# kevlar-dev/kevlar

Measured on AMD Instinct MI355X. Metric: reads/sec through count+novel (3 samples, k=31), higher is better.
Workload: dtype u64 hash / u8 counters

## Files before the change

kevlar_amd/csrc/kv_skm_bucket_device.h:

```cpp
#pragma once
#include "kv_skm_emit_device.h"

#define SKM_MAX_ABL 8
struct SkmAblSet {
    int n, ctrl_max;
    const uint64_t *keys[SKM_MAX_ABL];
    const uint8_t *cnts[SKM_MAX_ABL];
    const uint32_t *bstart[SKM_MAX_ABL], *bcount[SKM_MAX_ABL];
    uint32_t maxv[SKM_MAX_ABL];
};

namespace {

#define SKM_THREADS3 512
#define SKM_BUCKETS_PER_TICKET 8u
#define SKM_MAXPROBE 48
#define SKM_LOOSE_WGS 1024

#define SKM_STEP_MASK 62u
#define SKM_PROBE_STEP(h) ((((h) >> 20) & SKM_STEP_MASK) | 1u)
template <int TS>
__device__ __forceinline__ uint32_t skm_slot0(uint32_t sh) { return (TS & (TS - 1)) == 0 ? sh & (uint32_t)(TS - 1) : __umulhi(sh, (uint32_t)TS); }
template <int TS>
__device__ __forceinline__ uint32_t skm_step_of(uint32_t sh) { return (TS & (TS - 1)) == 0 ? SKM_PROBE_STEP(sh) : (((sh >> 2) & 62u) | 1u); }
template <int TS>
__device__ __forceinline__ uint32_t skm_slot_next(uint32_t slot, uint32_t step)
{
    if ((TS & (TS - 1)) == 0) return (slot + step) & (uint32_t)(TS - 1);
    slot += step;
    return slot >= (uint32_t)TS ? slot - (uint32_t)TS : slot;
}
template <int KW, int TS>
struct SkmTable {
    unsigned long long key[KW][TS];
};

template <int KW, int TS>
__device__ __forceinline__ void skm_table_clear(SkmTable<KW, TS> &tb)
{
    for (uint32_t i = threadIdx.x; i < TS; i += blockDim.x) {
        tb.key[0][i] = SKM_EMPTY;
        if (KW == 2) tb.key[KW - 1][i] = SKM_EMPTY;
    }
}

template <int KW, int TS>
__device__ __forceinline__ int skm_table_insert(SkmTable<KW, TS> &tb, const SkmKey<KW> &c)
{
    const uint32_t sh = skm_slot_hash<KW>(c);
    uint32_t slot = skm_slot0<TS>(sh);
    const uint32_t step = skm_step_of<TS>(sh);
    for (int probe = 0; probe < SKM_MAXPROBE; ++probe) {
        const unsigned long long old0 = atomicCAS(&tb.key[0][slot], SKM_EMPTY, (unsigned long long)c.w[0]);
        if (old0 == SKM_EMPTY || old0 == c.w[0]) {
            if (KW == 1) return (int)slot;
            const unsigned long long old1 = atomicCAS(&tb.key[KW - 1][slot], SKM_EMPTY, (unsigned long long)c.w[KW - 1]);
            if (old1 == SKM_EMPTY || old1 == c.w[KW - 1]) return (int)slot;
        }
        slot = skm_slot_next<TS>(slot, step);
    }
    return -1;
}

template <int KW, int TS>
__device__ __forceinline__ int skm_table_find(const SkmTable<KW, TS> &tb, const SkmKey<KW> &c)
{
    const uint32_t sh = skm_slot_hash<KW>(c);
    uint32_t slot = skm_slot0<TS>(sh);
    const uint32_t step = skm_step_of<TS>(sh);
    for (int probe = 0; probe < SKM_MAXPROBE; ++probe) {
        const unsigned long long k0 = tb.key[0][slot];
        if (k0 == SKM_EMPTY) return -1;
        if (k0 == c.w[0] && (KW == 1 || tb.key[KW - 1][slot] == c.w[KW - 1])) return (int)slot;
        slot = skm_slot_next<TS>(slot, step);
    }
    return -1;
}

template <int KW, int TS>
__device__ __forceinline__ SkmKey<KW> skm_table_key(const SkmTable<KW, TS> &tb, uint32_t slot)
{
    SkmKey<KW> c;
    c.w[0] = tb.key[0][slot];
    if (KW == 2) c.w[KW - 1] = tb.key[KW - 1][slot];
    return c;
}
template <int KW, int TS>
__device__ __forceinline__ SkmKey<KW> skm_table_take(SkmTable<KW, TS> &tb, uint32_t slot)
{
    const SkmKey<KW> c = skm_table_key(tb, slot);
    tb.key[0][slot] = SKM_EMPTY;
    if (KW == 2) tb.key[KW - 1][slot] = SKM_EMPTY;
    return c;
}

template <int KW>
__device__ __forceinline__ SkmKey<KW> skm_key_load(const uint64_t *keys, uint64_t e, bool live = true)
{
    SkmKey<KW> c;
    c.w[0] = live ? keys[e * KW] : SKM_EMPTY;
    if (KW == 2) c.w[KW - 1] = live ? keys[e * KW + (KW - 1)] : SKM_EMPTY;
    return c;
}
template <int KW>
__device__ __forceinline__ void skm_key_store(uint64_t *keys, uint64_t e, const SkmKey<KW> &c)
{
    keys[e * KW] = c.w[0];
    if (KW == 2) keys[e * KW + (KW - 1)] = c.w[KW - 1];
}
// ... 37 lines not shown
}

template <int TS, typename Body>
__device__ __forceinline__ void skm_for_occupied(const unsigned long long *key0, uint16_t *queue_all, uint32_t queue_stride, Body body, const uint32_t *skip = nullptr)
{
    const uint32_t wave = threadIdx.x >> 6, lane = threadIdx.x & 63, nwaves = blockDim.x >> 6;
    uint16_t *queue = queue_all + wave * queue_stride;
    const uint32_t per_wave = TS / nwaves;
    const uint32_t s_end = (wave + 1) * per_wave;
    uint32_t qn = 0;
    for (uint32_t s0 = wave * per_wave;; s0 += 64) {
        const bool last = s0 >= s_end;
        if (!last) {
            const uint32_t slot = s0 + lane;
            const bool occ = key0[slot] != SKM_EMPTY && !(skip && ((skip[slot >> 5] >> (slot & 31u)) & 1u));
            const unsigned long long ballot = __ballot(occ);
            if (occ) __hip_atomic_store(&queue[qn + (uint32_t)__popcll(ballot & ((1ull << lane) - 1ull))], (uint16_t)slot, __ATOMIC_RELAXED, __HIP_MEMORY_SCOPE_WAVEFRONT);
            qn += (uint32_t)__popcll(ballot);
            __builtin_amdgcn_fence(__ATOMIC_ACQ_REL, "wavefront");
            __builtin_amdgcn_wave_barrier();
        }
        if (qn >= 64 || (last && qn > 0)) {
            const uint32_t take = min(qn, 64u);
            qn -= take;
            if (lane < take) body((uint32_t)__hip_atomic_load(&queue[qn + lane], __ATOMIC_RELAXED, __HIP_MEMORY_SCOPE_WAVEFRONT));
            __builtin_amdgcn_fence(__ATOMIC_ACQ_REL, "wavefront");
            __builtin_amdgcn_wave_barrier();
        }
        if (last) break;
    }
}

#define SKM_UNIT 4

__device__ __forceinline__ uint64_t skm_shfl64(uint64_t v, uint32_t src)
{
    const uint32_t lo = (uint32_t)__shfl((int)(uint32_t)v, (int)src), hi = (uint32_t)__shfl((int)(uint32_t)(v >> 32), (int)src);
    return (uint64_t)lo | ((uint64_t)hi << 32);
}

template <int KW, bool WANT_POS>
__device__ __forceinline__ void skm_walk_loose(const SkmGeom &sg, bool alone, const SkmKey<KW> &kmer, uint64_t hdr, uint32_t owner,
                                               uint64_t pos0, uint32_t j0, uint32_t u, uint32_t lane, int recw)
{
    const unsigned long long need = __ballot(alone);
    if (!need) return;
    const uint64_t posu = WANT_POS ? pos0 : skm_hdr_pos_of(skm_shfl64(hdr, owner), j0 + u);
    unsigned long long first = 0;
    if (lane == 0) first = atomicAdd(&sg.ctr[SKM_CTR_LOOSE], (unsigned long long)__popcll(need));
    first = skm_shfl64(first, 0);
    if (alone) {
        const unsigned long long idx = first + (unsigned long long)__popcll(need & ((1ull << lane) - 1ull));
        uint64_t one[3] = {kmer.w[0], KW == 2 ? kmer.w[KW - 1] : 0ull, 0ull};
        if (idx < sg.loose_cap) skm_store_record(sg.loose + idx * (uint64_t)recw, skm_header(posu, 1u, 0u), one, sg.nbw);
        else sg.ctr[SKM_CTR_FAIL] = 1;
    }
}

template <int KW, bool WANT_POS, int FK = 0, bool COMPACT = false, typename Body>
__device__ __forceinline__ void skm_walk_bucket(const SkmGeom &sg, uint32_t b, uint32_t *sbits_all, Body body)
{
    static_assert(!COMPACT || (KW == 1 && !WANT_POS), "compact records: one-word keys, no positions");
    constexpr uint32_t G = SKM_UNIT;
    const uint32_t lane = threadIdx.x & 63, wave = threadIdx.x >> 6, nwaves = blockDim.x >> 6;
    uint32_t *sbits = sbits_all + wave * sg.sbw;
    const int k = FK ? FK : sg.k, recw = COMPACT ? 2 : (FK ? 1 + KW + 1 : sg.recw);
    auto load = [&](const uint64_t *rec, uint64_t &hdr, uint64_t &b0, uint64_t &b1, uint64_t &b2) {
        if (COMPACT) {
            typedef uint64_t u64x2a __attribute__((ext_vector_type(2), aligned(16)));
            const u64x2a both = *(const u64x2a *)rec;
            b0 = both.x; b1 = skm_c_b1(both.y); hdr = skm_header(0ull, skm_c_n(both.y), 0u, skm_c_rev(both.y));
        } else {
            hdr = rec[0]; b0 = rec[1]; b1 = rec[2];
            if (KW == 2) b2 = rec[3];
        }
    };
    const uint32_t *cnt2 = sg.cnt2 + (uint64_t)b * sg.nwg2;
    uint32_t p = wave;
    uint32_t g = p / sg.nwg2, sgm = p - g * sg.nwg2;
    uint64_t hdr = 0, b0 = 0, b1 = 0, b2 = 0;
    {
        const uint32_t at = min(g * 64u + lane, sg.cap2 - 1u);
        const uint64_t *rec = sg.seg2 + (((uint64_t)b * sg.nwg2 + sgm) * sg.cap2 + at) * (uint64_t)recw;
        load(rec, hdr, b0, b1, b2);
    }
    uint32_t maxc = 0;
    for (uint32_t s2 = 0; s2 < sg.nwg2; ++s2) maxc = max(maxc, cnt2[s2]);
    for (;;) {
        if (g * 64u >= maxc) break;
        const uint32_t NR = cnt2[sgm], i = g * 64u + lane;
        const uint32_t nk = i < NR ? skm_hdr_n(hdr) : 0u;
        const uint32_t nu = (nk + G - 1u) / G;
        uint32_t incl = nu;
#pragma unroll
        for (int d = 1; d < 64; d <<= 1) {
            const uint32_t up = __shfl_up(incl, d);
            if (lane >= d) incl += up;
        }
        const uint32_t total = __shfl(incl, 63), excl = incl - nu;
        const uint32_t exnk = excl | (nk << 16);
        const uint32_t nwords = (total >> 5) + 2u;
        for (uint32_t wd = lane; wd < nwords; wd += 64) sbits[wd] = 0;
        __builtin_amdgcn_fence(__ATOMIC_RELEASE, "wavefront");
        __builtin_amdgcn_wave_barrier();
        if (nu) atomicOr(&sbits[excl >> 5], 1u << (excl & 31));
        __builtin_amdgcn_fence(__ATOMIC_ACQ_REL, "wavefront");
        __builtin_amdgcn_wave_barrier();
        uint32_t before = 0;
        for (uint32_t t0 = 0; t0 < total; t0 += 64) {
            const uint64_t starts = (uint64_t)__hip_atomic_load(&sbits[t0 >> 5], __ATOMIC_RELAXED, __HIP_MEMORY_SCOPE_WAVEFRONT) |
                                    ((uint64_t)__hip_atomic_load(&sbits[(t0 >> 5) + 1], __ATOMIC_RELAXED, __HIP_MEMORY_SCOPE_WAVEFRONT) << 32);
            const uint32_t t = t0 + lane;
            const uint32_t owner = (before + (uint32_t)__popcll(starts & ((2ull << lane) - 1ull)) - 1u) & 63u;
            before += (uint32_t)__popcll(starts);
            const uint32_t oe = (uint32_t)__shfl((int)exnk, (int)owner);
            const uint64_t o0 = skm_shfl64(b0, owner), o1 = skm_shfl64(b1, owner);
            const uint64_t o2 = KW == 2 ? skm_shfl64(b2, owner) : 0ull;
            const uint64_t oh = WANT_POS ? skm_shfl64(hdr, owner) : 0ull;
            const uint32_t j0 = t < total ? (t - (oe & 0xffffu)) * G : 0u;
            const uint32_t cnt = t < total ? min(G, (oe >> 16) - j0) : 0u;
            SkmKey<KW> fw = skm_kmer_of<KW>(o0, o1, o2, j0, k);
            const uint32_t tail = (uint32_t)skm_window64(o0, o1, o2, j0 + (uint32_t)k);
            uint64_t pos0 = 0;
            int step = 1;
            if (WANT_POS) {
                const bool rv = skm_hdr_rev(oh) != 0u;
                pos0 = skm_hdr_pos(oh) + (rv ? skm_hdr_n(oh) - 1u - j0 : j0);
                step = rv ? -1 : 1;
            }
#pragma unroll
            for (uint32_t u = 0; u < G; ++u) {
                if (u) { SkmKey<KW> other = fw; skm_roll<KW>(fw, other, (tail >> (2u * (u - 1u))) & 3u, k); }
                const uint64_t posu = pos0 + (uint64_t)(int64_t)(step * (int)u);
                bool alone = false;
                if (u < cnt) alone = body(fw, posu);
                skm_walk_loose<KW, WANT_POS>(sg, alone, fw, hdr, owner, posu, j0, u, lane, sg.lrecw);
            }
        }
        __builtin_amdgcn_wave_barrier();
        p += nwaves;
        g = p / sg.nwg2; sgm = p - g * sg.nwg2;
        if (g * 64u >= maxc) break;
        if (g * 64u + lane < cnt2[sgm]) {
            const uint64_t *rec = sg.seg2 + (((uint64_t)b * sg.nwg2 + sgm) * sg.cap2 + g * 64u + lane) * (uint64_t)recw;
            load(rec, hdr, b0, b1, b2);
        }
    }
}

template <int CTR>
__device__ __forceinline__ uint32_t skm_first_bucket(const SkmGeom &sg) { return (uint32_t)atomicAdd(&sg.ctr[CTR], 1ull) * sg.bpt; }

template <int CTR, bool FAIL_ENDS, bool ESTIMATE>
__device__ __forceinline__ void skm_next_bucket(const SkmGeom &sg, uint32_t b, uint32_t taken, uint32_t &next)
{
    if ((b + 1u) & (sg.bpt - 1u)) next = b + 1u;
    else if (taken + 1 >= sg.quota3 || (FAIL_ENDS && __hip_atomic_load(&sg.ctr[SKM_CTR_FAIL], __ATOMIC_RELAXED, __HIP_MEMORY_SCOPE_AGENT) != 0)) next = 0xffffffffu;
    else {
        const unsigned long long ticket = atomicAdd(&sg.ctr[CTR], 1ull);
        next = (uint32_t)ticket * sg.bpt;
        if (ESTIMATE) {
            const unsigned long long done = ticket * sg.bpt;
            if (done * 50ull >= sg.n_buckets) {
                const unsigned long long now = __hip_atomic_load(&sg.ctr[SKM_CTR_LOOSE], __ATOMIC_RELAXED, __HIP_MEMORY_SCOPE_AGENT), start = sg.ctr[SKM_CTR_LOOSE_S12];
                if (now > start && (now - start) * 25ull > done * sg.bucket_kmers) sg.ctr[SKM_CTR_FAIL] = 1;
            }
        }
    }
}

__device__ __forceinline__ uint64_t skm_loose_len(const SkmGeom &sg)
{
    const unsigned long long n = sg.ctr[SKM_CTR_LOOSE];
    return n > sg.loose_cap ? sg.loose_cap : n;
}

template <int KW, typename Body>
__device__ __forceinline__ void skm_loose_walk_wave(const SkmGeom &sg, Body body)
{
    const unsigned long long n = skm_loose_len(sg);
// ... 2 lines not shown
    const uint64_t total_waves = (uint64_t)gridDim.x * (blockDim.x >> 6), wave_id = (uint64_t)blockIdx.x * (blockDim.x >> 6) + (threadIdx.x >> 6);
    const uint32_t per = (uint32_t)min((unsigned long long)64, max((unsigned long long)1, (n + total_waves - 1) / total_waves));
    for (uint64_t i0 = wave_id * per; i0 < n; i0 += total_waves * per) {
        const uint64_t i = i0 + lane;
        const bool have = lane < per && i < n;
        const uint64_t *rec = sg.loose + (have ? i : 0) * (uint64_t)sg.lrecw;
        uint64_t bw[3];
#pragma unroll
        for (int t = 0; t < 3; ++t) bw[t] = (have && t < sg.nbw) ? rec[1 + t] : 0ull;
        const uint64_t hdr = have ? rec[0] : 0ull;
        const uint32_t nk = skm_hdr_n(hdr);
        body(skm_first_kmer<KW>(bw, k), nk == 1, hdr, 0u);
        unsigned long long longer = __ballot(nk > 1);
        while (longer) {
            const uint32_t src = (uint32_t)__ffsll((long long)longer) - 1u;
            longer &= longer - 1ull;
            const uint64_t b0 = skm_shfl64(bw[0], src), b1 = skm_shfl64(bw[1], src), b2 = skm_shfl64(bw[2], src), h_src = skm_shfl64(hdr, src);
            const uint32_t nk_src = (uint32_t)__shfl((int)nk, (int)src);
            for (uint32_t j0 = 0; j0 < nk_src; j0 += 64) {
                const uint32_t j = j0 + lane;
                const bool live = j < nk_src;
                body(skm_kmer_of<KW>(b0, b1, b2, live ? j : 0u, k), live, h_src, live ? j : 0u);
            }
        }
    }
}

__host__ __device__ inline uint32_t skm_wave_scratch_words(uint32_t sbw) { return sbw > 64u ? sbw : 64u; }

#define SKM_K2_WAVES 6
#define SKM_TS51 2560
#define SKM_TS31 4096
#define SKM_LIST_MAX 4096u
template <int KW, int TS, bool FORCE_LOOSE, int FK, bool COMPACT = false>
__global__ __launch_bounds__(SKM_THREADS3, KW == 2 ? SKM_K2_WAVES : 6) void k_skm_count(SkmGeom sg, const SketchDev *__restrict__ sk,
                                                           const SketchDev *__restrict__ mask, ConsumeFilter f, BinGeom g)
{
    static_assert((uint32_t)TS <= SKM_LIST_MAX, "a bucket's distinct list (one entry per occupied slot) must fit what k_skm_novel_list takes");
    constexpr bool PL = FK != 0;
    __shared__ SkmTable<KW, TS> tb;
    __shared__ uint32_t cnt[PL ? TS / 2 : TS];
    __shared__ uint32_t next_bucket;
    __shared__ uint32_t abl_cur, abl_b0, abl_prev;
    __shared__ uint32_t dl_cur, dl_b0;
    extern __shared__ __attribute__((aligned(16))) uint32_t dyn[];
    const uint32_t ns = (uint32_t)(g.T * g.C);
    uint32_t *lut = dyn, *cur = dyn + (PL ? 1024 : 256), *scratch = cur + ((ns + 3u) & ~3u);
    uint64_t *P1 = (uint64_t *)dyn, *P2 = P1 + 256;
    for (uint32_t s = threadIdx.x; s < ns; s += SKM_THREADS3) cur[s] = 0;
    if (threadIdx.x < 256) {
        if (PL) { P1[threadIdx.x] = skm_ascii4_times(threadIdx.x, MM_C1); P2[threadIdx.x] = skm_ascii4_times(threadIdx.x, MM_C2); }
        else lut[threadIdx.x] = skm_ascii4(threadIdx.x);
    }
    const HashParams hp = FK ? make_hash_params(FK, f.hp.hashfam) : f.hp;
    uint64_t n_added = 0, n_distinct = 0;
    const uint32_t cap1 = (uint32_t)g.cap1;
    uint32_t *my_seg = g.gbuf1 + (uint64_t)blockIdx.x * g.cap1;
    const uint64_t seg_stride = (uint64_t)g.nwgA * g.cap1;
    auto emit = [&](int t, uint64_t bin, uint32_t wgt) {
        const uint32_t slice = (uint32_t)(bin >> g.sbits);
        const uint32_t c = g.F == 1 ? slice : __umulhi(slice, g.recipF);
        const uint32_t sidx = (uint32_t)t * (uint32_t)g.C + c;
        const uint32_t item = ((slice - c * (uint32_t)g.F) << g.sbits) | ((uint32_t)bin & ((1u << g.sbits) - 1u)) | ((wgt - 1u) << BIN_W_SHIFT);
        const uint32_t pos = atomicAdd(&cur[sidx], 1u);
        if (pos < cap1) my_seg[sidx * seg_stride + pos] = item;
        else spill_item(g, t, bin, wgt);
    };
    skm_table_clear(tb);
    for (uint32_t i = threadIdx.x; i < (PL ? TS / 2 : TS); i += SKM_THREADS3) cnt[i] = 0;
    if (threadIdx.x == 0) { next_bucket = skm_first_bucket<SKM_CTR_TICKET_COUNT>(sg); abl_cur = 0; abl_b0 = 0; abl_prev = 0xffffffffu; dl_cur = 0; dl_b0 = 0; }
    auto abl_close = [&]() {
        if (sg.abl_keys && abl_prev != 0xffffffffu) {
            const bool fits = abl_cur <= sg.abl_cap_wg;
            sg.abl_bstart[abl_prev] = blockIdx.x * sg.abl_cap_wg + abl_b0;
            sg.abl_bcount[abl_prev] = fits ? abl_cur - abl_b0 : 0u;
        }
        if (sg.dl_keys && abl_prev != 0xffffffffu) {
            sg.dl_bstart[abl_prev] = blockIdx.x * sg.dl_cap_wg + dl_b0;
            sg.dl_bcount[abl_prev] = dl_cur - dl_b0;
        }
    };
    for (uint32_t taken = 0; taken < sg.quota3; ++taken) {
        __syncthreads();
        const uint32_t b = next_bucket;
        if (b >= sg.n_buckets) break;
        __syncthreads();
        if (threadIdx.x == 0) {
            abl_close();
            abl_prev = b; abl_b0 = abl_cur; dl_b0 = dl_cur;
            skm_next_bucket<SKM_CTR_TICKET_COUNT, true, true>(sg, b, taken, next_bucket);
        }
        skm_walk_bucket<KW, false, FK, COMPACT>(sg, b, scratch, [&](const SkmKey<KW> &c, uint64_t) {
            const bool forced = FORCE_LOOSE && sg.force_loose && ((c.w[0] * 0x9e3779b97f4a7c15ull) >> 58) == 0;
            const int slot = skm_cacheable<KW>(c) && !forced ? skm_table_insert(tb, c) : -1;
            if (slot >= 0) {
                if (PL) atomicAdd(&cnt[(uint32_t)slot >> 1], 1u << (((uint32_t)slot & 1u) * 16u));
                else atomicAdd(&cnt[slot], 1u);
            }
            return slot < 0;
        });
        __syncthreads();
        skm_for_occupied<TS>(tb.key[0], (uint16_t *)scratch, skm_wave_scratch_words(sg.sbw) * 2u, [&](uint32_t slot) {
            const SkmKey<KW> c = skm_table_take(tb, slot);
            uint32_t seen;
            if (PL) {
                const uint32_t sh = (slot & 1u) * 16u;
                seen = (cnt[slot >> 1] >> sh) & 0xffffu;
                atomicSub(&cnt[slot >> 1], seen << sh);
            } else {
                seen = cnt[slot];
                cnt[slot] = 0;
            }
            n_distinct += 1;
            uint64_t h;
            if constexpr (PL) h = skm_key_hash_pl<KW, FK>(c, P1, P2);
            else h = skm_key_hash<KW>(c, lut, hp);
            if (sg.dl_keys) skm_dl_push<KW>(sg, &dl_cur, (uint64_t)blockIdx.x * sg.dl_cap_wg, sg.dl_cap_wg, c, h);
            uint32_t added;
            if (g.fast4 && !f.use_mask) {
                const bool pass = !f.use_band || (h >= f.band_lo && h < f.band_hi);
                added = pass ? seen : 0u;
                if (pass) {
                    const double hd = kv_fastmod_hd(h);
                    uint32_t bin[4];
#pragma unroll
                    for (int t = 0; t < 4; ++t) bin[t] = kv_fastmod32(h, hd, (uint32_t)g.tsize[t], g.tmagic[t]);
                    uint32_t left = min(seen, 255u);
                    const uint32_t omask = (1u << g.sbits) - 1u, stride32 = (uint32_t)seg_stride;
                    while (left) {
                        const uint32_t wgt = min(left, BIN_W_MAX), wbits = (wgt - 1u) << BIN_W_SHIFT;
#pragma unroll
                        for (int t = 0; t < 4; ++t) {
                            const uint32_t slice = bin[t] >> g.sbits;
                            const uint32_t c = g.F == 1 ? slice : __umulhi(slice, g.recipF);
                            const uint32_t sidx = (uint32_t)t * (uint32_t)g.C + c;
                            const uint32_t item = ((slice - c * (uint32_t)g.F) << g.sbits) | (bin[t] & omask) | wbits;
                            const uint32_t pos = atomicAdd(&cur[sidx], 1u);
                            if (pos < cap1) my_seg[sidx * stride32 + pos] = item;
                            else spill_item(g, t, (uint64_t)bin[t], wgt);
                        }
                        left -= wgt;
                    }
                }
            } else {
                added = skm_count_kmer(h, seen, sk, mask, f, g.T, emit);
            }
            n_added += added;
            if (sg.abl_keys) {
                const bool want = added >= 2u;
                const uint32_t at = skm_wave_reserve(&abl_cur, want);
                if (want && at < sg.abl_cap_wg) {
                    const uint64_t e = (uint64_t)blockIdx.x * sg.abl_cap_wg + at;
                    skm_key_store<KW>(sg.abl_keys, e, c);
                    sg.abl_cnts[e] = (uint8_t)min(added, 255u);
                }
            }
        });
    }
    __syncthreads();
    if (threadIdx.x == 0) {
        abl_close();
        if (sg.dl_keys && dl_cur > sg.dl_cap_wg) atomicAdd(&sg.ctr[SKM_CTR_DL_RAN_OUT], 1ull);
    }
    for (uint32_t s = threadIdx.x; s < ns; s += SKM_THREADS3)
        g.gcnt1[(uint64_t)s * g.nwgA + blockIdx.x] = (uint32_t)min((uint64_t)cur[s], g.cap1);
    n_added = wave_sum_u64(n_added);
    n_distinct = wave_sum_u64(n_distinct);
    if ((threadIdx.x & 63) == 0 && n_added) atomicAdd(&g.ctr[BIN_CTR_ADDED], (unsigned long long)n_added);
    if ((threadIdx.x & 63) == 0 && n_distinct) atomicAdd(&sg.ctr[SKM_CTR_DISTINCT], (unsigned long long)n_distinct);
}

template <int KW>
__global__ __launch_bounds__(256) void k_skm_loose_count(SkmGeom sg, const SketchDev *__restrict__ sk,
                                                         const SketchDev *__restrict__ mask, ConsumeFilter f, BinGeom g)
{
    __shared__ uint32_t lut[256];
    if (sg.ctr[SKM_CTR_FAIL] != 0) return;
    lut[threadIdx.x] = skm_ascii4(threadIdx.x);
    __syncthreads();
    const int k = sg.k;
    uint64_t n_added = 0;
    skm_loose_walk_wave<KW>(sg, [&](const SkmKey<KW> &fw, bool live, uint64_t, uint32_t) {
        uint64_t h = 0;
        bool pass = false;
        if (live) {
            h = skm_key_hash<KW>(skm_canonical<KW>(fw, skm_revcomp<KW>(fw, k)), lut, f.hp);
            pass = consume_filter_pass(f, mask, h);
// ... 514 lines not shown
```

kevlar_amd/csrc/kv_skm.hip:

```cpp
#include <algorithm>
#include <cmath>

#include "kv_binned.h"
#include "kv_novel_device.h"
#include "kv_skm_device.h"
#include "kv_skm_emit_device.h"
#include "kv_skm_bucket_device.h"

namespace {

template <typename F> KvInst<F> skm_inst(F *fn, const char *name) { return kv_inst(fn, name); }
#define SKM_INST(...) skm_inst(__VA_ARGS__, #__VA_ARGS__)
KvPerStream<KvLaunched> g_skm_launched;
void skm_launched_begin(hipStream_t st) { g_skm_launched.get(st).begin(); }
template <typename F> F *skm_launching(const KvInst<F> &k, hipStream_t st)
{
    g_skm_launched.get(st).note(k.name);
    return k.fn;
}

struct SkmCarve {
    unsigned char *base;
    size_t total = 0;
    explicit SkmCarve(void *arena = nullptr) : base((unsigned char *)arena) {}
// ... 441 lines not shown
                if (al.mem) (void)hipFree(al.mem);
                al.mem = nullptr; al.bytes = 0;
                if (kv_hip_malloc(&al.mem, need) == hipSuccess) al.bytes = need;
                else (void)hipGetLastError();
            }
            if (al.mem) {
                skm_list_lay(SkmCarve(al.mem), cap_wg * nwg3, sg.kw, sg.n_buckets, &al.keys, &al.cnts, &al.bstart, &al.bcount);
                KV_HIP(skm_list_zero(al.bstart, al.bcount, st));
                al.k = k; al.m = sg.m; al.kw = sg.kw; al.C1 = sg.C1; al.F2 = sg.F2; al.fbits = sg.fbits; al.n_buckets = sg.n_buckets;
                al.nwg = nwg3; al.cap_wg = cap_wg; al.cap_total = cap_wg * nwg3;
                skm_abl_attach(al, sg);
                abl_new = true;
            }
        }
    }
    bool dl_new = false;
    const char *dl_env = kv_knob("KV_SKM_DL");
    if (s->scan_hint && !(dl_env && atoi(dl_env) == 0)) {
        const double frac = std::min(1.0, std::max(0.3, s->skm_distinct * 1.15));
        const uint64_t cap_wg = std::min<uint64_t>((uint64_t)((double)n_kmers * frac * 1.6 / nwg3) + 4096, 0xfffffff0ull / nwg3);
        const bool worth = (dl_env && atoi(dl_env) == 1) || s->scan_steady || idx.builds > 1 || idx.dl.bytes >= SkmDistinctList::bytes(cap_wg * nwg3, sg.kw, sg.n_buckets);
        const int lrc = worth ? idx.list.carve(idx.dl, cap_wg * nwg3, sg.kw, sg.n_buckets, (uint32_t)cap_wg, 0, 0, st) : KV_ERR_CAPACITY;
        if (lrc != KV_OK && lrc != KV_ERR_CAPACITY) return lrc;
        if (lrc == KV_OK) { idx.list.attach(sg); dl_new = true; }
        else (void)hipGetLastError();
    }
    {
        KvProfScope prof("k_skm_count");
        const uint32_t ns = (uint32_t)(plan.g.T * plan.g.C);
        const bool fixed_k = !sg.force_loose && !kv_knob("KV_SKM_ANY_K") && (uint64_t)sg.nwg2 * sg.cap2 * (uint64_t)sg.ncap < 65536ull;
        auto kernel = sg.kw == 1 ? (sg.force_loose ? SKM_INST(k_skm_count<1, 4096, true, 0>) : SKM_INST(k_skm_count<1, 4096, false, 0>))
                                 : (sg.force_loose ? SKM_INST(k_skm_count<2, 2048, true, 0>) : SKM_INST(k_skm_count<2, 2048, false, 0>));
        bool pl = false;
        if (sg.k == 31 && sg.recw == 3 && fixed_k) { kernel = SKM_INST(k_skm_count<1, SKM_TS31, false, 31>); pl = true; }
        if (sg.compact) {
            kernel = sg.force_loose ? SKM_INST(k_skm_count<1, 4096, true, 0, true>) : SKM_INST(k_skm_count<1, 4096, false, 0, true>);
            pl = false;
            if (sg.k == 31 && fixed_k) { kernel = SKM_INST(k_skm_count<1, SKM_TS31, false, 31, true>); pl = true; }
        }
        if (sg.k == 51 && sg.recw == 4 && fixed_k) { kernel = SKM_INST(k_skm_count<2, SKM_TS51, false, 51>); pl = true; }
        const size_t lds = ((pl ? 1024 : 256) + ((ns + 3u) & ~3u) + (size_t)(SKM_THREADS3 / 64) * skm_wave_scratch_words(sg.sbw)) * 4;
        hipLaunchKernelGGL(skm_launching(kernel, st), dim3(nwg3), dim3(SKM_THREADS3), lds, st, sg, (const SketchDev *)s->d_desc, d_mask, filter, plan.g);
    }
    {
        KvProfScope prof("k_skm_loose_count");
        skm_launch_loose(SKM_INST(k_skm_loose_count<1>), SKM_INST(k_skm_loose_count<2>), st, sg, s->d_desc, d_mask, filter, plan.g);
    }
    KV_HIP(hipGetLastError());
    hipLaunchKernelGGL(k_skm_forward_flag, dim3(1), dim3(1), 0, st, sg.ctr, plan.g.ctr);
    KV_HIP(hipGetLastError());
    skm_abl_detach(sg);
    SkmDistinctList::detach(sg);
    const int rc = kv_bin_finish(s, plan, true, 0, n_added);
    if (abl_new) s->abl.valid = rc == KV_OK;
    {
        unsigned long long sc[SKM_CTR_DL_RAN_OUT + 1] = {0};
        const bool got = hipMemcpy(sc, sg.ctr, sizeof(sc), hipMemcpyDeviceToHost) == hipSuccess;
        idx.dl_valid = dl_new && got && rc == KV_OK && sc[SKM_CTR_DL_RAN_OUT] == 0;
        if (dl_new && kv_knob("KV_SKM_VERBOSE")) fprintf(stderr, "[kv_skm] distinct list: %s (%llu workgroups ran out of %u entries)\n", idx.dl_valid ? "kept" : "dropped", sc[SKM_CTR_DL_RAN_OUT], idx.list.cap_wg);
        if (got && n_kmers) {
            const double alone = skm_outside_tables(sc) / (double)n_kmers;
            const double distinct = (double)sc[SKM_CTR_DISTINCT] / (double)n_kmers + alone;
            s->skm_off = rc != KV_OK || alone > 0.03 || distinct > 0.45;
            s->skm_off_kmers = (distinct > 0.45 || rc == KV_ERR_CAPACITY) ? n_kmers : 0;
            s->skm_distinct = distinct;
            { std::lock_guard<std::mutex> glk(g_skm_mu); g_skm_last_distinct = distinct; }
            if (kv_knob("KV_SKM_VERBOSE"))
                fprintf(stderr, "[kv_skm] batch of %llu k-mers: %.1f%% distinct, %.2f%% outside the LDS tables, %llu of %llu records (%d bytes each) outside their segments%s\n",
                        (unsigned long long)n_kmers, 100 * distinct, 100 * alone, sc[SKM_CTR_LOOSE_S12], sc[SKM_CTR_RECORDS], 8 * sg.recw,
                        s->skm_off ? " -> next batches take the plain partition" : "");
        }
    }
    if (rc != KV_OK) {
        idx.drop(SkmIndex::BATCH | SkmIndex::MEX_SCAN);
// ... 480 lines not shown
```

Before: 1.060 billion.

## Re-read kernel arguments from kernarg segment to cut register pressure; unroll probes

Inside the per-bucket loops the kernel now gets a fresh pointer to its kernarg segment, hidden behind an empty asm barrier. Geometry, filter and bin fields are then reloaded as scalar loads instead of being kept live in registers across the whole kernel. The hash-table insert and find loops are rewritten with a single exit and an explicit clang unroll count. The aim is to lower SGPR/VGPR pressure and spills at the 6-waves launch bound and to let probes issue back to back. The cost is that it depends on the argument block layout matching a hand-written struct, which is checked only by a static_assert.

```diff
diff --git a/kevlar_amd/csrc/kv_skm_bucket_device.h b/kevlar_amd/csrc/kv_skm_bucket_device.h
--- a/kevlar_amd/csrc/kv_skm_bucket_device.h
+++ b/kevlar_amd/csrc/kv_skm_bucket_device.h
@@ -1,4 +1,5 @@
 #pragma once
+#include <cstddef>
 #include "kv_skm_emit_device.h"
 
 #define SKM_MAX_ABL 8
@@ -15,6 +16,7 @@
 #define SKM_THREADS3 512
 #define SKM_BUCKETS_PER_TICKET 8u
 #define SKM_MAXPROBE 48
+#define SKM_PROBE_UNROLL(KW) ((KW) == 1 ? 8 : 4)
 #define SKM_LOOSE_WGS 1024
 
 #define SKM_STEP_MASK 62u
@@ -50,16 +52,19 @@
     const uint32_t sh = skm_slot_hash<KW>(c);
     uint32_t slot = skm_slot0<TS>(sh);
     const uint32_t step = skm_step_of<TS>(sh);
+    int at = -1;
+#pragma clang loop unroll_count(SKM_PROBE_UNROLL(KW))
     for (int probe = 0; probe < SKM_MAXPROBE; ++probe) {
         const unsigned long long old0 = atomicCAS(&tb.key[0][slot], SKM_EMPTY, (unsigned long long)c.w[0]);
-        if (old0 == SKM_EMPTY || old0 == c.w[0]) {
-            if (KW == 1) return (int)slot;
+        bool mine = old0 == SKM_EMPTY || old0 == c.w[0];
+        if (KW == 2 && mine) {
             const unsigned long long old1 = atomicCAS(&tb.key[KW - 1][slot], SKM_EMPTY, (unsigned long long)c.w[KW - 1]);
-            if (old1 == SKM_EMPTY || old1 == c.w[KW - 1]) return (int)slot;
-        }
+            mine = old1 == SKM_EMPTY || old1 == c.w[KW - 1];
+        }
+        if (mine) { at = (int)slot; break; }
         slot = skm_slot_next<TS>(slot, step);
     }
-    return -1;
+    return at;
 }
 
 template <int KW, int TS>
@@ -68,13 +73,15 @@
     const uint32_t sh = skm_slot_hash<KW>(c);
     uint32_t slot = skm_slot0<TS>(sh);
     const uint32_t step = skm_step_of<TS>(sh);
+    int at = -1;
+#pragma clang loop unroll_count(SKM_PROBE_UNROLL(KW))
     for (int probe = 0; probe < SKM_MAXPROBE; ++probe) {
         const unsigned long long k0 = tb.key[0][slot];
-        if (k0 == SKM_EMPTY) return -1;
-        if (k0 == c.w[0] && (KW == 1 || tb.key[KW - 1][slot] == c.w[KW - 1])) return (int)slot;
+        if (k0 == SKM_EMPTY) break;
+        if (k0 == c.w[0] && (KW == 1 || tb.key[KW - 1][slot] == c.w[KW - 1])) { at = (int)slot; break; }
         slot = skm_slot_next<TS>(slot, step);
     }
-    return -1;
+    return at;
 }
 
 template <int KW, int TS>
@@ -360,6 +367,18 @@
 #define SKM_TS51 2560
 #define SKM_TS31 4096
 #define SKM_LIST_MAX 4096u
+struct SkmCountArgs { SkmGeom sg; const SketchDev *sk, *mask; ConsumeFilter f; BinGeom g; };
+static_assert(alignof(SkmGeom) == 8 && alignof(ConsumeFilter) == 8 && alignof(BinGeom) == 8 &&
+              offsetof(SkmCountArgs, g) == sizeof(SkmGeom) + 2 * sizeof(void *) + sizeof(ConsumeFilter),
+              "SkmCountArgs must lie as k_skm_count's argument block does");
+template <typename Args>
+__device__ __forceinline__ const Args *skm_args_again()
+{
+    typedef const __attribute__((address_space(4))) Args *ArgsPtr;
+    ArgsPtr p = (ArgsPtr)__builtin_amdgcn_kernarg_segment_ptr();
+    asm volatile("" : "+s"(p));
+    return (const Args *)p;
+}
 template <int KW, int TS, bool FORCE_LOOSE, int FK, bool COMPACT = false>
 __global__ __launch_bounds__(SKM_THREADS3, KW == 2 ? SKM_K2_WAVES : 6) void k_skm_count(SkmGeom sg, const SketchDev *__restrict__ sk,
                                                            const SketchDev *__restrict__ mask, ConsumeFilter f, BinGeom g)
@@ -418,8 +437,9 @@
             abl_prev = b; abl_b0 = abl_cur; dl_b0 = dl_cur;
             skm_next_bucket<SKM_CTR_TICKET_COUNT, true, true>(sg, b, taken, next_bucket);
         }
-        skm_walk_bucket<KW, false, FK, COMPACT>(sg, b, scratch, [&](const SkmKey<KW> &c, uint64_t) {
-            const bool forced = FORCE_LOOSE && sg.force_loose && ((c.w[0] * 0x9e3779b97f4a7c15ull) >> 58) == 0;
+        const SkmGeom &sw = skm_args_again<SkmCountArgs>()->sg;
+        skm_walk_bucket<KW, false, FK, COMPACT>(sw, b, scratch, [&](const SkmKey<KW> &c, uint64_t) {
+            const bool forced = FORCE_LOOSE && sw.force_loose && ((c.w[0] * 0x9e3779b97f4a7c15ull) >> 58) == 0;
             const int slot = skm_cacheable<KW>(c) && !forced ? skm_table_insert(tb, c) : -1;
             if (slot >= 0) {
                 if (PL) atomicAdd(&cnt[(uint32_t)slot >> 1], 1u << (((uint32_t)slot & 1u) * 16u));
@@ -428,6 +448,10 @@
             return slot < 0;
         });
         __syncthreads();
+        const SkmCountArgs &ka = *skm_args_again<SkmCountArgs>();
+        const SkmGeom &sd = ka.sg; const ConsumeFilter &fd = ka.f; const BinGeom &gd = ka.g;
+        const uint32_t cap1d = (uint32_t)gd.cap1, stride32 = (uint32_t)((uint64_t)gd.nwgA * gd.cap1);
+        uint32_t *seg_d = gd.gbuf1 + (uint64_t)blockIdx.x * gd.cap1;
         skm_for_occupied<TS>(tb.key[0], (uint16_t *)scratch, skm_wave_scratch_words(sg.sbw) * 2u, [&](uint32_t slot) {
             const SkmKey<KW> c = skm_table_take(tb, slot);
             uint32_t seen;
@@ -443,29 +467,29 @@
             uint64_t h;
             if constexpr (PL) h = skm_key_hash_pl<KW, FK>(c, P1, P2);
             else h = skm_key_hash<KW>(c, lut, hp);
-            if (sg.dl_keys) skm_dl_push<KW>(sg, &dl_cur, (uint64_t)blockIdx.x * sg.dl_cap_wg, sg.dl_cap_wg, c, h);
+            if (sd.dl_keys) skm_dl_push<KW>(sd, &dl_cur, (uint64_t)blockIdx.x * sd.dl_cap_wg, sd.dl_cap_wg, c, h);
             uint32_t added;
-            if (g.fast4 && !f.use_mask) {
-                const bool pass = !f.use_band || (h >= f.band_lo && h < f.band_hi);
+            if (gd.fast4 && !fd.use_mask) {
+                const bool pass = !fd.use_band || (h >= fd.band_lo && h < fd.band_hi);
                 added = pass ? seen : 0u;
                 if (pass) {
                     const double hd = kv_fastmod_hd(h);
                     uint32_t bin[4];
 #pragma unroll
-                    for (int t = 0; t < 4; ++t) bin[t] = kv_fastmod32(h, hd, (uint32_t)g.tsize[t], g.tmagic[t]);
+                    for (int t = 0; t < 4; ++t) bin[t] = kv_fastmod32(h, hd, (uint32_t)gd.tsize[t], gd.tmagic[t]);
                     uint32_t left = min(seen, 255u);
-                    const uint32_t omask = (1u << g.sbits) - 1u, stride32 = (uint32_t)seg_stride;
+                    const uint32_t omask = (1u << gd.sbits) - 1u;
                     while (left) {
                         const uint32_t wgt = min(left, BIN_W_MAX), wbits = (wgt - 1u) << BIN_W_SHIFT;
 #pragma unroll
                         for (int t = 0; t < 4; ++t) {
-                            const uint32_t slice = bin[t] >> g.sbits;
-                            const uint32_t c = g.F == 1 ? slice : __umulhi(slice, g.recipF);
-                            const uint32_t sidx = (uint32_t)t * (uint32_t)g.C + c;
-                            const uint32_t item = ((slice - c * (uint32_t)g.F) << g.sbits) | (bin[t] & omask) | wbits;
+                            const uint32_t slice = bin[t] >> gd.sbits;
+                            const uint32_t c = gd.F == 1 ? slice : __umulhi(slice, gd.recipF);
+                            const uint32_t sidx = (uint32_t)t * (uint32_t)gd.C + c;
+                            const uint32_t item = ((slice - c * (uint32_t)gd.F) << gd.sbits) | (bin[t] & omask) | wbits;
                             const uint32_t pos = atomicAdd(&cur[sidx], 1u);
-                            if (pos < cap1) my_seg[sidx * stride32 + pos] = item;
-                            else spill_item(g, t, (uint64_t)bin[t], wgt);
+                            if (pos < cap1d) seg_d[sidx * stride32 + pos] = item;
+                            else spill_item(gd, t, (uint64_t)bin[t], wgt);
                         }
                         left -= wgt;
                     }
@@ -474,13 +498,13 @@
                 added = skm_count_kmer(h, seen, sk, mask, f, g.T, emit);
             }
             n_added += added;
-            if (sg.abl_keys) {
+            if (sd.abl_keys) {
                 const bool want = added >= 2u;
                 const uint32_t at = skm_wave_reserve(&abl_cur, want);
-                if (want && at < sg.abl_cap_wg) {
-                    const uint64_t e = (uint64_t)blockIdx.x * sg.abl_cap_wg + at;
-                    skm_key_store<KW>(sg.abl_keys, e, c);
-                    sg.abl_cnts[e] = (uint8_t)min(added, 255u);
+                if (want && at < sd.abl_cap_wg) {
+                    const uint64_t e = (uint64_t)blockIdx.x * sd.abl_cap_wg + at;
+                    skm_key_store<KW>(sd.abl_keys, e, c);
+                    sd.abl_cnts[e] = (uint8_t)min(added, 255u);
                 }
             }
         });
```

Measured after the change: 1.068 billion, median of 4. About the same (+0.7%).

## Combine duplicate compact super-k-mer records before k-mer insertion in count kernel

Applied to the files above, without the earlier changes.

For the k=31 compact-record path, each bucket's two-word records are first deduplicated in a record hash table that overlays the k-mer table in LDS, and each copy count becomes a weight. The walk then compacts away duplicate records per wave and inserts each distinct record's k-mers once, adding the weight to the counter. This targets the repeated LDS atomic inserts caused by identical reads at high coverage. In exchange it adds a pre-pass with atomics, extra syncs and more LDS, and falls back to unweighted walking when a bucket has more than two 64-record groups per wave or the record table overflows.

```diff
diff --git a/kevlar_amd/csrc/kv_skm.hip b/kevlar_amd/csrc/kv_skm.hip
--- a/kevlar_amd/csrc/kv_skm.hip
+++ b/kevlar_amd/csrc/kv_skm.hip
@@ -497,14 +497,16 @@
         auto kernel = sg.kw == 1 ? (sg.force_loose ? SKM_INST(k_skm_count<1, 4096, true, 0>) : SKM_INST(k_skm_count<1, 4096, false, 0>))
                                  : (sg.force_loose ? SKM_INST(k_skm_count<2, 2048, true, 0>) : SKM_INST(k_skm_count<2, 2048, false, 0>));
         bool pl = false;
+        bool rc = false;
         if (sg.k == 31 && sg.recw == 3 && fixed_k) { kernel = SKM_INST(k_skm_count<1, SKM_TS31, false, 31>); pl = true; }
         if (sg.compact) {
             kernel = sg.force_loose ? SKM_INST(k_skm_count<1, 4096, true, 0, true>) : SKM_INST(k_skm_count<1, 4096, false, 0, true>);
             pl = false;
-            if (sg.k == 31 && fixed_k) { kernel = SKM_INST(k_skm_count<1, SKM_TS31, false, 31, true>); pl = true; }
+            if (sg.k == 31 && fixed_k) { kernel = SKM_INST(k_skm_count<1, SKM_TS31, false, 31, true>); pl = true; rc = true; }
         }
         if (sg.k == 51 && sg.recw == 4 && fixed_k) { kernel = SKM_INST(k_skm_count<2, SKM_TS51, false, 51>); pl = true; }
-        const size_t lds = ((pl ? 1024 : 256) + ((ns + 3u) & ~3u) + (size_t)(SKM_THREADS3 / 64) * skm_wave_scratch_words(sg.sbw)) * 4;
+        const size_t lds = ((pl ? 1024 : 256) + ((ns + 3u) & ~3u) + (size_t)(SKM_THREADS3 / 64) * skm_wave_scratch_words(sg.sbw)) * 4 +
+                           (rc ? SKM_RC_LDS_WORDS * 4 : 0);
         hipLaunchKernelGGL(skm_launching(kernel, st), dim3(nwg3), dim3(SKM_THREADS3), lds, st, sg, (const SketchDev *)s->d_desc, d_mask, filter, plan.g);
     }
     {
diff --git a/kevlar_amd/csrc/kv_skm_bucket_device.h b/kevlar_amd/csrc/kv_skm_bucket_device.h
--- a/kevlar_amd/csrc/kv_skm_bucket_device.h
+++ b/kevlar_amd/csrc/kv_skm_bucket_device.h
@@ -1,4 +1,6 @@
 #pragma once
+#include <cstddef>
+#include <type_traits>
 #include "kv_skm_emit_device.h"
 
 #define SKM_MAX_ABL 8
@@ -45,7 +47,7 @@
 }
 
 template <int KW, int TS>
-__device__ __forceinline__ int skm_table_insert(SkmTable<KW, TS> &tb, const SkmKey<KW> &c)
+__device__ __forceinline__ int skm_table_insert(SkmTable<KW, TS> &tb, const SkmKey<KW> &c, bool *claimed = nullptr)
 {
     const uint32_t sh = skm_slot_hash<KW>(c);
     uint32_t slot = skm_slot0<TS>(sh);
@@ -53,9 +55,15 @@
     for (int probe = 0; probe < SKM_MAXPROBE; ++probe) {
         const unsigned long long old0 = atomicCAS(&tb.key[0][slot], SKM_EMPTY, (unsigned long long)c.w[0]);
         if (old0 == SKM_EMPTY || old0 == c.w[0]) {
-            if (KW == 1) return (int)slot;
+            if (KW == 1) {
+                if (claimed) *claimed = old0 == SKM_EMPTY;
+                return (int)slot;
+            }
             const unsigned long long old1 = atomicCAS(&tb.key[KW - 1][slot], SKM_EMPTY, (unsigned long long)c.w[KW - 1]);
-            if (old1 == SKM_EMPTY || old1 == c.w[KW - 1]) return (int)slot;
+            if (old1 == SKM_EMPTY || old1 == c.w[KW - 1]) {
+                if (claimed) *claimed = old1 == SKM_EMPTY;
+                return (int)slot;
+            }
         }
         slot = skm_slot_next<TS>(slot, step);
     }
@@ -178,6 +186,12 @@
 }
 
 #define SKM_UNIT 4
+#define SKM_RC_GROUPS 2u
+#define SKM_RC_LDS_WORDS ((SKM_THREADS3 / 64) * SKM_RC_GROUPS * 64u / 2u + 4u)
+struct SkmRecWeights {
+    const uint16_t *all;
+    bool hold;
+};
 
 __device__ __forceinline__ uint64_t skm_shfl64(uint64_t v, uint32_t src)
 {
@@ -185,13 +199,32 @@
     return (uint64_t)lo | ((uint64_t)hi << 32);
 }
 
-template <int KW, bool WANT_POS>
+template <int KW, bool WANT_POS, bool WEIGHTED = false>
 __device__ __forceinline__ void skm_walk_loose(const SkmGeom &sg, bool alone, const SkmKey<KW> &kmer, uint64_t hdr, uint32_t owner,
-                                               uint64_t pos0, uint32_t j0, uint32_t u, uint32_t lane, int recw)
+                                               uint64_t pos0, uint32_t j0, uint32_t u, uint32_t lane, int recw, uint32_t wt = 1u)
 {
     const unsigned long long need = __ballot(alone);
     if (!need) return;
     const uint64_t posu = WANT_POS ? pos0 : skm_hdr_pos_of(skm_shfl64(hdr, owner), j0 + u);
+    if constexpr (WEIGHTED) {
+        const uint32_t mine = alone ? wt : 0u;
+        uint32_t incl = mine;
+#pragma unroll
+        for (int d = 1; d < 64; d <<= 1) {
+            const uint32_t up = __shfl_up(incl, d);
+            if (lane >= (uint32_t)d) incl += up;
+        }
+        const uint32_t total = __shfl(incl, 63);
+        unsigned long long first = 0;
+        if (lane == 0) first = atomicAdd(&sg.ctr[SKM_CTR_LOOSE], (unsigned long long)total);
+        first = skm_shfl64(first, 0) + (incl - mine);
+        uint64_t one[3] = {kmer.w[0], KW == 2 ? kmer.w[KW - 1] : 0ull, 0ull};
+        for (uint32_t c = 0; c < mine; ++c) {
+            if (first + c < sg.loose_cap) skm_store_record(sg.loose + (first + c) * (uint64_t)recw, skm_header(posu, 1u, 0u), one, sg.nbw);
+            else sg.ctr[SKM_CTR_FAIL] = 1;
+        }
+        return;
+    }
     unsigned long long first = 0;
     if (lane == 0) first = atomicAdd(&sg.ctr[SKM_CTR_LOOSE], (unsigned long long)__popcll(need));
     first = skm_shfl64(first, 0);
@@ -203,12 +236,16 @@
     }
 }
 
-template <int KW, bool WANT_POS, int FK = 0, bool COMPACT = false, typename Body>
-__device__ __forceinline__ void skm_walk_bucket(const SkmGeom &sg, uint32_t b, uint32_t *sbits_all, Body body)
+template <int KW, bool WANT_POS, int FK = 0, bool COMPACT = false, typename Body, typename Wts = std::nullptr_t>
+__device__ __forceinline__ void skm_walk_bucket(const SkmGeom &sg, uint32_t b, uint32_t *sbits_all, Body body, Wts wts = nullptr)
 {
     static_assert(!COMPACT || (KW == 1 && !WANT_POS), "compact records: one-word keys, no positions");
+    constexpr bool WEIGHTED = !std::is_same<Wts, std::nullptr_t>::value;
+    static_assert(!WEIGHTED || COMPACT, "weights: compact records (n < 64, so at most 1024 units in front of a record: exnk below)");
     constexpr uint32_t G = SKM_UNIT;
-    const uint32_t lane = threadIdx.x & 63, wave = threadIdx.x >> 6, nwaves = blockDim.x >> 6;
+    uint32_t tid = threadIdx.x;
+    if constexpr (WEIGHTED) asm volatile("" : "+v"(tid));
+    const uint32_t lane = tid & 63, wave = tid >> 6, nwaves = blockDim.x >> 6;
     uint32_t *sbits = sbits_all + wave * sg.sbw;
     const int k = FK ? FK : sg.k, recw = COMPACT ? 2 : (FK ? 1 + KW + 1 : sg.recw);
     auto load = [&](const uint64_t *rec, uint64_t &hdr, uint64_t &b0, uint64_t &b1, uint64_t &b2) {
@@ -232,10 +269,30 @@
     }
     uint32_t maxc = 0;
     for (uint32_t s2 = 0; s2 < sg.nwg2; ++s2) maxc = max(maxc, cnt2[s2]);
-    for (;;) {
+    for (uint32_t r = 0;; ++r) {
         if (g * 64u >= maxc) break;
         const uint32_t NR = cnt2[sgm], i = g * 64u + lane;
-        const uint32_t nk = i < NR ? skm_hdr_n(hdr) : 0u;
+        uint32_t wt = 1u;
+        bool live = i < NR;
+        if constexpr (WEIGHTED) {
+            if (wts.hold) {
+                wt = wts.all[(wave * SKM_RC_GROUPS + r) * 64u + lane];
+                const unsigned long long keep = __ballot(live && wt != 0u);
+                uint16_t *from = (uint16_t *)sbits;
+                if (live && wt != 0u)
+                    __hip_atomic_store(&from[__builtin_amdgcn_mbcnt_hi((uint32_t)(keep >> 32), __builtin_amdgcn_mbcnt_lo((uint32_t)keep, 0u))], (uint16_t)lane,
+                                       __ATOMIC_RELAXED, __HIP_MEMORY_SCOPE_WAVEFRONT);
+                __builtin_amdgcn_fence(__ATOMIC_ACQ_REL, "wavefront");
+                __builtin_amdgcn_wave_barrier();
+                live = lane < (uint32_t)__popcll(keep);
+                const uint32_t src = live ? (uint32_t)__hip_atomic_load(&from[lane], __ATOMIC_RELAXED, __HIP_MEMORY_SCOPE_WAVEFRONT) : lane;
+                __builtin_amdgcn_fence(__ATOMIC_ACQ_REL, "wavefront");
+                __builtin_amdgcn_wave_barrier();
+                hdr = skm_shfl64(hdr, src); b0 = skm_shfl64(b0, src); b1 = skm_shfl64(b1, src);
+                wt = (uint32_t)__shfl((int)wt, (int)src);
+            }
+        }
+        const uint32_t nk = live ? skm_hdr_n(hdr) : 0u;
         const uint32_t nu = (nk + G - 1u) / G;
         uint32_t incl = nu;
 #pragma unroll
@@ -244,7 +301,7 @@
             if (lane >= d) incl += up;
         }
         const uint32_t total = __shfl(incl, 63), excl = incl - nu;
-        const uint32_t exnk = excl | (nk << 16);
+        const uint32_t exnk = WEIGHTED ? excl | (nk << 10) | (wt << 16) : excl | (nk << 16);
         const uint32_t nwords = (total >> 5) + 2u;
         for (uint32_t wd = lane; wd < nwords; wd += 64) sbits[wd] = 0;
         __builtin_amdgcn_fence(__ATOMIC_RELEASE, "wavefront");
@@ -263,8 +320,8 @@
             const uint64_t o0 = skm_shfl64(b0, owner), o1 = skm_shfl64(b1, owner);
             const uint64_t o2 = KW == 2 ? skm_shfl64(b2, owner) : 0ull;
             const uint64_t oh = WANT_POS ? skm_shfl64(hdr, owner) : 0ull;
-            const uint32_t j0 = t < total ? (t - (oe & 0xffffu)) * G : 0u;
-            const uint32_t cnt = t < total ? min(G, (oe >> 16) - j0) : 0u;
+            const uint32_t j0 = t < total ? (t - (oe & (WEIGHTED ? 0x3ffu : 0xffffu))) * G : 0u;
+            const uint32_t cnt = t < total ? min(G, (WEIGHTED ? (oe >> 10) & 63u : oe >> 16) - j0) : 0u;
             SkmKey<KW> fw = skm_kmer_of<KW>(o0, o1, o2, j0, k);
             const uint32_t tail = (uint32_t)skm_window64(o0, o1, o2, j0 + (uint32_t)k);
             uint64_t pos0 = 0;
@@ -279,8 +336,13 @@
                 if (u) { SkmKey<KW> other = fw; skm_roll<KW>(fw, other, (tail >> (2u * (u - 1u))) & 3u, k); }
                 const uint64_t posu = pos0 + (uint64_t)(int64_t)(step * (int)u);
                 bool alone = false;
-                if (u < cnt) alone = body(fw, posu);
-                skm_walk_loose<KW, WANT_POS>(sg, alone, fw, hdr, owner, posu, j0, u, lane, sg.lrecw);
+                if constexpr (WEIGHTED) {
+                    if (u < cnt) alone = body(fw, posu, oe >> 16);
+                    skm_walk_loose<KW, WANT_POS, true>(sg, alone, fw, hdr, owner, posu, j0, u, lane, sg.lrecw, oe >> 16);
+                } else {
+                    if (u < cnt) alone = body(fw, posu);
+                    skm_walk_loose<KW, WANT_POS>(sg, alone, fw, hdr, owner, posu, j0, u, lane, sg.lrecw);
+                }
             }
         }
         __builtin_amdgcn_wave_barrier();
@@ -292,6 +354,64 @@
             load(rec, hdr, b0, b1, b2);
         }
     }
+}
+
+#define SKM_RC_NONE 0xffffu
+#define SKM_RC_SELF 0xfffeu
+template <int TS>
+__device__ __forceinline__ bool skm_combine_records(const SkmGeom &sg, uint32_t b, SkmTable<1, TS> &tb, uint32_t *cnt, uint16_t *wts_all, uint32_t *fail)
+{
+    typedef SkmTable<2, TS / 2> RecTable;
+    static_assert(sizeof(RecTable) == sizeof(SkmTable<1, TS>) && TS / 2 < (int)SKM_RC_SELF, "the record table lies over the k-mer table");
+    RecTable &rt = reinterpret_cast<RecTable &>(tb);
+    uint32_t tid = threadIdx.x;
+    asm volatile("" : "+v"(tid));
+    const uint32_t lane = tid & 63, wave = tid >> 6, nwaves = blockDim.x >> 6;
+    const uint32_t *cnt2 = sg.cnt2 + (uint64_t)b * sg.nwg2;
+    uint32_t maxc = 0;
+    for (uint32_t s2 = 0; s2 < sg.nwg2; ++s2) maxc = max(maxc, cnt2[s2]);
+    if (sg.nwg2 * ((maxc + 63u) >> 6) > SKM_RC_GROUPS * nwaves) return false;
+    uint16_t *wts = wts_all + wave * (SKM_RC_GROUPS * 64u) + lane;
+#pragma unroll 1
+    for (uint32_t r = 0; r < SKM_RC_GROUPS; ++r) {
+        const uint32_t p = wave + r * nwaves, g = p / sg.nwg2, sgm = p - g * sg.nwg2, i = g * 64u + lane;
+        uint32_t note = SKM_RC_NONE;
+        if (i < cnt2[sgm]) {
+            typedef uint64_t u64x2a __attribute__((ext_vector_type(2), aligned(16)));
+            const u64x2a both = *(const u64x2a *)(sg.seg2 + (((uint64_t)b * sg.nwg2 + sgm) * sg.cap2 + i) * 2u);
+            SkmKey<2> rec;
+            rec.w[0] = both.x; rec.w[1] = both.y;
+            note = SKM_RC_SELF;
+            if (skm_cacheable<2>(rec)) {
+                bool mine = false;
+                const int slot = skm_table_insert(rt, rec, &mine);
+                if (slot < 0) *fail = 1u;
+                else {
+                    atomicAdd(&cnt[(uint32_t)slot >> 1], 1u << (((uint32_t)slot & 1u) * 16u));
+                    note = mine ? (uint32_t)slot : SKM_RC_NONE;
+                }
+            }
+        }
+        wts[r * 64u] = (uint16_t)note;
+    }
+    __syncthreads();
+    const bool holds = __builtin_amdgcn_readfirstlane((int)*fail) == 0;
+#pragma unroll 1
+    for (uint32_t r = 0; r < SKM_RC_GROUPS; ++r) {
+        const uint32_t note = wts[r * 64u];
+        uint32_t wt = note == SKM_RC_SELF ? 1u : 0u;
+        if (note < SKM_RC_SELF) {
+            const uint32_t sh = (note & 1u) * 16u;
+            wt = (cnt[note >> 1] >> sh) & 0xffffu;
+            atomicSub(&cnt[note >> 1], wt << sh);
+            rt.key[0][note] = SKM_EMPTY;
+            rt.key[1][note] = SKM_EMPTY;
+        }
+        wts[r * 64u] = (uint16_t)wt;
+    }
+    __syncthreads();
+    if (tid == 0) *fail = 0u;
+    return holds;
 }
 
 template <int CTR>
@@ -366,6 +486,7 @@
 {
     static_assert((uint32_t)TS <= SKM_LIST_MAX, "a bucket's distinct list (one entry per occupied slot) must fit what k_skm_novel_list takes");
     constexpr bool PL = FK != 0;
+    constexpr bool RC = PL && COMPACT && KW == 1;
     __shared__ SkmTable<KW, TS> tb;
     __shared__ uint32_t cnt[PL ? TS / 2 : TS];
     __shared__ uint32_t next_bucket;
@@ -373,8 +494,11 @@
     __shared__ uint32_t dl_cur, dl_b0;
     extern __shared__ __attribute__((aligned(16))) uint32_t dyn[];
     const uint32_t ns = (uint32_t)(g.T * g.C);
-    uint32_t *lut = dyn, *cur = dyn + (PL ? 1024 : 256), *scratch = cur + ((ns + 3u) & ~3u);
+    uint32_t *lut = dyn, *cur = dyn + (PL ? 1024 : 256) + (RC ? SKM_RC_LDS_WORDS : 0), *scratch = cur + ((ns + 3u) & ~3u);
     uint64_t *P1 = (uint64_t *)dyn, *P2 = P1 + 256;
+    uint16_t *rc_wts = (uint16_t *)(dyn + 1024);
+    uint32_t *rc_fail = dyn + 1024 + SKM_RC_LDS_WORDS - 4;
+    if (RC && threadIdx.x == 0) *rc_fail = 0u;
     for (uint32_t s = threadIdx.x; s < ns; s += SKM_THREADS3) cur[s] = 0;
     if (threadIdx.x < 256) {
         if (PL) { P1[threadIdx.x] = skm_ascii4_times(threadIdx.x, MM_C1); P2[threadIdx.x] = skm_ascii4_times(threadIdx.x, MM_C2); }
@@ -418,15 +542,21 @@
             abl_prev = b; abl_b0 = abl_cur; dl_b0 = dl_cur;
             skm_next_bucket<SKM_CTR_TICKET_COUNT, true, true>(sg, b, taken, next_bucket);
         }
-        skm_walk_bucket<KW, false, FK, COMPACT>(sg, b, scratch, [&](const SkmKey<KW> &c, uint64_t) {
+        auto combine = [&](const SkmKey<KW> &c, uint32_t wt) {
             const bool forced = FORCE_LOOSE && sg.force_loose && ((c.w[0] * 0x9e3779b97f4a7c15ull) >> 58) == 0;
             const int slot = skm_cacheable<KW>(c) && !forced ? skm_table_insert(tb, c) : -1;
             if (slot >= 0) {
-                if (PL) atomicAdd(&cnt[(uint32_t)slot >> 1], 1u << (((uint32_t)slot & 1u) * 16u));
-                else atomicAdd(&cnt[slot], 1u);
+                if (PL) atomicAdd(&cnt[(uint32_t)slot >> 1], wt << (((uint32_t)slot & 1u) * 16u));
+                else atomicAdd(&cnt[slot], wt);
             }
             return slot < 0;
-        });
+        };
+        if constexpr (RC) {
+            const SkmRecWeights wts = {rc_wts, skm_combine_records<TS>(sg, b, tb, cnt, rc_wts, rc_fail)};
+            skm_walk_bucket<KW, false, FK, COMPACT>(sg, b, scratch, [&](const SkmKey<KW> &c, uint64_t, uint32_t wt) { return combine(c, wt); }, wts);
+        } else {
+            skm_walk_bucket<KW, false, FK, COMPACT>(sg, b, scratch, [&](const SkmKey<KW> &c, uint64_t) { return combine(c, 1u); });
+        }
         __syncthreads();
         skm_for_occupied<TS>(tb.key[0], (uint16_t *)scratch, skm_wave_scratch_words(sg.sbw) * 2u, [&](uint32_t slot) {
             const SkmKey<KW> c = skm_table_take(tb, slot);
diff --git a/scratch/record_copies_groups.py b/scratch/record_copies_groups.py
--- /dev/null
+++ b/scratch/record_copies_groups.py
@@ -0,0 +1,59 @@
+import collections
+import numpy as np
+
+rng = np.random.default_rng(5)
+G, L, k, m, cov, err, ncap, per_bucket = 200_000, 100, 31, 12, 30, 0.005, 34, 890
+w = k - m + 1
+genome = rng.integers(0, 4, G, dtype=np.uint8)
+n = cov * G // L
+starts = rng.integers(0, G - L, n)
+reads = genome[starts[:, None] + np.arange(L)[None, :]]
+rev = rng.integers(0, 2, n).astype(bool)
+reads[rev] = 3 - reads[rev][:, ::-1]
+e = rng.random((n, L)) < err
+reads = np.where(e, (reads + rng.integers(1, 4, (n, L))) % 4, reads).astype(np.uint8)
+nm = L - m + 1
+f = np.zeros((n, nm), dtype=np.uint64); r = np.zeros((n, nm), dtype=np.uint64)
+for i in range(m):
+    f |= reads[:, i:i + nm].astype(np.uint64) << np.uint64(2 * i)
+    r |= (3 - reads[:, i:i + nm]).astype(np.uint64) << np.uint64(2 * (m - 1 - i))
+can = np.minimum(f, r)
+order = (can * np.uint64(0x9e3779b1)) & np.uint64(0xffffffff)
+order ^= order >> np.uint64(15)
+order = (order << np.uint64(1)) | (r < f).astype(np.uint64)
+nk = L - k + 1
+win = np.lib.stride_tricks.sliding_window_view(order, w, axis=1)
+minv = win.min(axis=2)
+change = np.ones((n, nk), dtype=bool); change[:, 1:] = minv[:, 1:] != minv[:, :-1]
+
+
+def rc(b):
+    return bytes(3 - x for x in reversed(b))
+
+
+records = []
+for i in range(n):
+    s = np.flatnonzero(change[i]); e2 = np.append(s[1:], nk)
+    row = reads[i].tobytes()
+    for a, b in zip(s, e2):
+        mv = int(minv[i, a])
+        while a < b:
+            ln = min(b - a, ncap)
+            rec = row[a:a + ln + k - 1]
+            records.append((mv >> 1, rc(rec) if mv & 1 else rec, ln))
+            a += ln
+n_buckets = max(1, len(records) // per_bucket)
+buckets = collections.defaultdict(list)
+for key, rec, ln in records:
+    buckets[(key * 0x9e3779b97f4a7c15 >> 20) % n_buckets].append((rec, ln))
+total = sum(ln for _, _, ln in records)
+print('records', len(records), 'k-mers', total, 'buckets', n_buckets, 'records per bucket', len(records) / n_buckets)
+print('| scope within which copies are combined | k-mer inserts left |')
+print('|---|---|')
+for scope, name in ((64, '64 records (one wave\'s group)'), (128, '128 records'), (0, 'the whole bucket')):
+    left = 0
+    for recs in buckets.values():
+        step = scope or len(recs)
+        for g0 in range(0, len(recs), step):
+            left += sum(ln for _, ln in set(recs[g0:g0 + step]))
+    print('| {} | {:.1f} % |'.format(name, 100.0 * left / total))
```

New measurement: 1.073 billion before, 1.049 billion after. -2.3%, worse.
